# dusk-network/dusk-blindbidproof

Hardware: AMD Instinct MI355X
Metric: blind-bid proofs/sec (higher is better)
Workload: dtype u32

## Files before the change

__graft_entry__.py:

```python
import os
import shutil
import subprocess
import sys

ROOT = os.path.dirname(os.path.abspath(__file__))
PKG = os.path.join(ROOT, "dusk_blindbidproof_amd")
CSRC = os.path.join(PKG, "csrc")
LIB = os.path.join(PKG, "libbbp_hip.so")
ORACLE_SO = os.path.join(ROOT, "oracle", "_build", "libbbp_oracle.so")
HOSTCHECK_SO = os.path.join(ROOT, "tests", "_build", "libhostcheck.so")
DEVCHECK_SO = {"chain": os.path.join(ROOT, "tests", "_build", "libbbp_devcheck.so"),
               "nochain": os.path.join(ROOT, "tests", "_build", "libbbp_devcheck_nochain.so")}
DEVCHECK_DEFS = {"chain": [], "nochain": ["-DBBP_FE_NO_CHAIN"]}


def _newer(target, sources):
    if not os.path.exists(target):
        return True
    t = os.path.getmtime(target)
    return any(os.path.getmtime(s) > t for s in sources)


def _run(cmd):
    print("+", " ".join(cmd), flush=True)
# ... 273 lines not shown
        _run(["g++", "-O1", "-g", "-std=c++17", "-fsanitize=address,undefined", "-fno-sanitize-recover=all", "-o", ROUND_STANDING_BIN, src])
    return ROUND_STANDING_BIN


ROUNDS_BEST_DISTINCT_BIN = os.path.join(ROOT, "tests", "_build", "rounds_best_distinct_check")


def build_rounds_best_distinct_check(force=False):
    src = os.path.join(ROOT, "tests", "rounds_best_distinct_check.cpp")
    if force or _newer(ROUNDS_BEST_DISTINCT_BIN, [src] + _csrc_files((".h", ".inc")) + [os.path.join(ROOT, "include", "bbp.h")]):
        os.makedirs(os.path.dirname(ROUNDS_BEST_DISTINCT_BIN), exist_ok=True)
        _run(["g++", "-O1", "-g", "-std=c++17", "-fsanitize=address,undefined", "-fno-sanitize-recover=all", "-o", ROUNDS_BEST_DISTINCT_BIN, src])
    return ROUNDS_BEST_DISTINCT_BIN


def build_secret_wipe_san(force=False):
    srcs = [os.path.join(ROOT, "tests", "secret_wipe_san.cpp"), os.path.join(CSRC, "submit.cpp")]
    if force or _newer(SECRET_WIPE_SAN_BIN, srcs + _csrc_files((".h", ".inc"))):
        os.makedirs(os.path.dirname(SECRET_WIPE_SAN_BIN), exist_ok=True)
        _run(["g++", "-O1", "-g", "-std=c++17", "-pthread", "-fsanitize=address,undefined", "-fno-sanitize-recover=all", "-o", SECRET_WIPE_SAN_BIN] + srcs)
    return SECRET_WIPE_SAN_BIN


STUB_ENTROPY_SO = os.path.join(ROOT, "tests", "_build", "libbbp_stub_entropy.so")


def build_stub_engine_entropy(force=False):
    srcs = [os.path.join(ROOT, "tests", "stub_engine_entropy.cpp"), os.path.join(CSRC, "submit.cpp")]
    if force or _newer(STUB_ENTROPY_SO, srcs + [os.path.join(ROOT, "tests", "stub_engine.cpp"), os.path.join(CSRC, "submit.h"), os.path.join(ROOT, "include", "bbp.h")]):
        os.makedirs(os.path.dirname(STUB_ENTROPY_SO), exist_ok=True)
# ... 51 lines not shown

def build():
    build_hip()
    build_server()
    build_stub_engine()
    build_oracle()
    build_hostcheck()
    build_sortcheck()
    build_roundcheck()
    build_round_select_check()
    build_round_best_check()
    build_round_best_distinct_check()
    build_rounds_best_check()
    build_rounds_best_distinct_check()
    build_round_standing_check()
    build_devcheck_all()
    sys.path.insert(0, ROOT)
    import dusk_blindbidproof_amd


def smoke():
    sys.path.insert(0, ROOT)
    import dusk_blindbidproof_amd as bbp
    from tests import smoke_case

    smoke_case.run(bbp)


if __name__ == "__main__":
    build()
# ... 1 lines not shown
```

dusk_blindbidproof_amd/csrc/msm.hip:

```cpp
#include "context.h"

namespace bbp {

#ifndef BBP_FOLD_PRIO
#define BBP_FOLD_PRIO 2
#endif
#ifndef BBP_MSM_WAVES
#define BBP_MSM_WAVES 2
#endif
#ifndef BBP_MSM_WAVES_MAX
#define BBP_MSM_WAVES_MAX 2
#endif

#ifdef BBP_MSM_PROF
__device__ unsigned long long g_msm_prof[8];
#define MSM_PROF_BEGIN() unsigned long long prof_t = wall_clock64()
#define MSM_PROF_MARK(i)                                                    \
    if (tid == 0) {                                                         \
        unsigned long long now_ = wall_clock64();                           \
        atomicAdd(&g_msm_prof[i], now_ - prof_t);                           \
        prof_t = now_;                                                      \
    }
#else
#define MSM_PROF_BEGIN()
// ... 60 lines not shown
    const u32 An = A ^ (neg << 6);
    const uint4 a0 = *reinterpret_cast<const uint4*>(wb + An), a1 = *reinterpret_cast<const uint4*>(wb + (An ^ 0x10u));
    const uint2 a2 = *reinterpret_cast<const uint2*>(wb + (An ^ 0x20u));
    const uint4 b0 = *reinterpret_cast<const uint4*>(wb + (An ^ 0x40u)), b1 = *reinterpret_cast<const uint4*>(wb + (An ^ 0x50u));
    const uint2 b2 = *reinterpret_cast<const uint2*>(wb + (An ^ 0x60u));
    const uint2 x0 = *reinterpret_cast<const uint2*>(wb + (A ^ 0x20u) + 8);
    const uint4 x1 = *reinterpret_cast<const uint4*>(wb + (A ^ 0x30u));
    const uint2 x2 = *reinterpret_cast<const uint2*>(wb + (A ^ 0x60u) + 8), x3 = *reinterpret_cast<const uint2*>(wb + (A ^ 0x70u));
    row_regs r;
    r.ypx = fe{{(i32)a0.x, (i32)a0.y, (i32)a0.z, (i32)a0.w, (i32)a1.x, (i32)a1.y, (i32)a1.z, (i32)a1.w, (i32)a2.x, (i32)a2.y}};
    r.ymx = fe{{(i32)b0.x, (i32)b0.y, (i32)b0.z, (i32)b0.w, (i32)b1.x, (i32)b1.y, (i32)b1.z, (i32)b1.w, (i32)b2.x, (i32)b2.y}};
    r.xy2d = fe{{(i32)x0.x, (i32)x0.y, (i32)x1.x, (i32)x1.y, (i32)x1.z, (i32)x1.w, (i32)x2.x, (i32)x2.y, (i32)x3.x, (i32)x3.y}};
    return r;
}
#endif

__device__ __noinline__ void ge_add_nc(ge& r, const ge& a, const ge& b) { r = ge_add(a, b); }
__device__ __noinline__ void ge_dbl_nc(ge& r, const ge& a) { r = ge_dbl(a); }

#ifndef BBP_SORT_T
#define BBP_SORT_T 1024
#endif
constexpr int SORT_T = BBP_SORT_T;
template <int MODE> struct msm_geom;
template <> struct msm_geom<0> { static constexpr int K = MSM_K, NAF = MSM_NAF, W = MSM_W; };
template <> struct msm_geom<1> { static constexpr int K = FOLD_K, NAF = FOLD_NAF, W = FOLD_W; };
template <> struct msm_geom<2> { static constexpr int K = SMALL_K, NAF = SMALL_NAF, W = SMALL_W; };

template <int MODE>
__global__ __launch_bounds__(SORT_T) void k_msm_sort(const u32* __restrict__ scal_a, const u32* __restrict__ aux, u32 n_total, u32 n_idx_sets,
                                                      u32 n_sub, u32 split, u32* __restrict__ sorted_all, u32* __restrict__ cursor_all,
                                                      const u32* __restrict__ msm_map, const u32* __restrict__ n_active, u32* __restrict__ ticket) {
    constexpr int K = msm_geom<MODE>::K, NAF = msm_geom<MODE>::NAF, W = msm_geom<MODE>::W, G = K >= SORT_T ? K / SORT_T : 1;
// ... 259 lines not shown
        __syncthreads();
    }
    u32* cur_out = cursor_all + work * (size_t)(K + 1);
    for (int k = tid; k <= K; k += SORT_T) cur_out[k] = k ? start[k + 1] : 0u;
}

#ifndef BBP_ACC_WG
#define BBP_ACC_WG 256
#endif
constexpr int ACC_WG = BBP_ACC_WG, ACC_WGS = ACC_T / ACC_WG;
static_assert(ACC_T % ACC_WG == 0 && ACC_WG % 64 == 0, "accumulate workgroup geometry");

template <int MODE>
__global__ __launch_bounds__(ACC_WG) __attribute__((amdgpu_waves_per_eu(BBP_MSM_WAVES, BBP_MSM_WAVES_MAX)))
void k_msm_acc(const niels_row* __restrict__ ptable, const u32* __restrict__ sorted_all, const u32* __restrict__ cursor_all, u32 n ,
               ge* __restrict__ bsum_all, ge* __restrict__ psum_all, ge* __restrict__ out, const u32* __restrict__ n_active, u32* __restrict__ fault,
               u32 n_work, u32* __restrict__ ticket) {
    constexpr int K = msm_geom<MODE>::K, W = msm_geom<MODE>::W, G = K / MSM_T;
    __shared__ u32 cursor[K + 1];
#ifdef BBP_ACC_PERSIST
    static_assert(ACC_WGS == 1, "the persistent form draws whole MSMs");
    __shared__ u32 s_ticket;
  for (;;) {
    __syncthreads();
    if (threadIdx.x == 0) s_ticket = atomicAdd(ticket, 1u);
    __syncthreads();
    const size_t msm = s_ticket;
    if (msm >= n_work || (n_active && msm >= *n_active)) return;
    const int tid = (int)threadIdx.x;
#else
    const size_t msm = blockIdx.x / ACC_WGS;
    const int tid = (int)(blockIdx.x % ACC_WGS) * ACC_WG + (int)threadIdx.x;
// ... 2 lines not shown
    const u32* sorted = sorted_all + msm * (size_t)n * W;
#ifdef BBP_MSM_PRIO
    __builtin_amdgcn_s_setprio(BBP_MSM_PRIO);
#endif
    MSM_PROF_BEGIN();
    {
        const u32* cur_in = cursor_all + msm * (size_t)(K + 1);
        for (int k = threadIdx.x; k <= K; k += ACC_WG) cursor[k] = cur_in[k];
    }
    __syncthreads();
    MSM_PROF_MARK(1);

    const u32 E = cursor[K];
    ge* bsum = bsum_all + msm * (size_t)K;
    ge* psum = psum_all + msm * (size_t)ACC_T;
#ifdef BBP_KO_ACC_PERMILLE
    const u32 c0 = (u32)(((u64)tid * E) / ACC_T), c1 = c0 + (u32)(((u64)((u32)(((u64)(tid + 1) * E) / ACC_T) - c0) * BBP_KO_ACC_PERMILLE) / 1000);
#else
    const u32 c0 = (u32)(((u64)tid * E) / ACC_T), c1 = (u32)(((u64)(tid + 1) * E) / ACC_T);
#endif
#ifdef BBP_MSM_PROF
    const unsigned long long clk0 = clock64();
#endif
    u32 k_first = 0;
    bool inside = false;
#ifdef BBP_ACC_COOP
    {
        __shared__ __attribute__((aligned(1024))) u8 rowimg[ACC_WG / 64][COOP_IMG];
        const int lane = (int)threadIdx.x & 63;
        u8* wb = rowimg[threadIdx.x >> 6];
// ... 1 lines not shown
        const u32 srcoff = (((u32)lane & 7u) ^ (((u32)lane >> 3) >> 1)) << 4;
        const u32 n_it = (E + (u32)ACC_T - 1) / (u32)ACC_T, len = c1 - c0;
        u32 k = 1, kend = 0;
        ge* dest = &psum[tid];
        if (len) {
            u32 lo = 1, hi = K;
            while (lo < hi) {
                u32 mid = (lo + hi) >> 1;
                if (cursor[mid] > c0) hi = mid; else lo = mid + 1;
            }
            k = lo, kend = cursor[k];
            k_first = lo;
            inside = cursor[k - 1] < c0;
            if (!inside) dest = &bsum[k - 1];
        }
        ge acc = ge_identity();
        u32 ent_cur = len ? sorted[c0] : 0u;
        u32 ent_nxt = len > 1 ? sorted[c0 + 1] : 0u;
        if (n_it) coop_issue(ptable, wb, coop_clamp_row(ent_cur, fault), lane, srcoff);
        for (u32 it = 0; it < n_it; it++) {
            const u32 e = c0 + it;
            const row_regs cur = coop_read(wb, A, ent_cur >> 31);
            const bool neg = ent_cur >> 31;
            ent_cur = ent_nxt;
            const bool live = it < len;
            if (live && e == kend) {
                *dest = acc;
                acc = ge_identity();
                do { k++; kend = cursor[k]; } while (kend == e);
                dest = &bsum[k - 1];
// ... 3 lines not shown
            if (it + 2 < len) ent_nxt = sorted[e + 2]; else ent_nxt = 0u;
            if (live) acc = ge_madd_row(acc, cur, neg);
        }
        if (len) *dest = acc;
    }
#else
    if (c0 < c1) {
        u32 lo = 1, hi = K;
        while (lo < hi) {
            u32 mid = (lo + hi) >> 1;
            if (cursor[mid] > c0) hi = mid; else lo = mid + 1;
        }
        u32 k = lo, kend = cursor[k];
        k_first = lo;
        inside = cursor[k - 1] < c0;
        ge* dest = inside ? &psum[tid] : &bsum[k - 1];
        ge acc = ge_identity();
        u32 ent_cur = sorted[c0];
        u32 ent_nxt = (c0 + 1 < c1) ? sorted[c0 + 1] : 0u;
        row_regs row = load_row(ptable, ent_cur, fault);
        for (u32 e = c0; e < c1; e++) {
            if (e == kend) {
                *dest = acc;
                acc = ge_identity();
                do { k++; kend = cursor[k]; } while (kend == e);
                dest = &bsum[k - 1];
            }
            const row_regs cur = row;
            const bool neg = ent_cur >> 31;
            ent_cur = ent_nxt;
            if (e + 1 < c1) row = load_row(ptable, ent_cur, fault);
            if (e + 2 < c1) ent_nxt = sorted[e + 2];
            acc = ge_madd_row(acc, cur, neg);
        }
        *dest = acc;
    }
#endif
#ifdef BBP_MSM_PROF
    if (tid == 0) atomicAdd(&g_msm_prof[6], clock64() - clk0);
#endif
    MSM_PROF_MARK(2);
    __threadfence_block();
    __syncthreads();
    MSM_PROF_MARK(3);
#ifdef BBP_ACC_PERSIST
  }
#endif
}

template <int MODE>
__global__ __launch_bounds__(MSM_T) void k_msm_fold(const u32* __restrict__ cursor_all, ge* __restrict__ bsum_all, const ge* __restrict__ psum_all,
                                                     ge* __restrict__ out, const u32* __restrict__ n_active) {
    constexpr int K = msm_geom<MODE>::K, G = K / MSM_T;
    __shared__ u32 cursor[K + 1];
    __shared__ u32 xch[GE_WORDS];
    const int tid = threadIdx.x;
    if (n_active && blockIdx.x >= *n_active) return;
    __builtin_amdgcn_s_setprio(BBP_FOLD_PRIO);
    const size_t msm = blockIdx.x;
    {
        const u32* cur_in = cursor_all + msm * (size_t)(K + 1);
        for (int k = tid; k <= K; k += MSM_T) cursor[k] = cur_in[k];
    }
    __syncthreads();
    const u32 E = cursor[K];
    ge* bsum = bsum_all + msm * (size_t)K;
    const ge* psum = psum_all + msm * (size_t)ACC_T;
#ifdef BBP_KO_FOLD
    if (MODE != 1) { if (tid == 0) out[msm] = bsum[0]; }
    else if (tid < FOLD_CLS) out[msm * FOLD_CLS + tid] = bsum[tid];
    return;
#endif
    for (u32 ch = tid; ch < (u32)ACC_T; ch += MSM_T) {
        const u32 c0 = (u32)(((u64)ch * E) / ACC_T), c1 = (u32)(((u64)(ch + 1) * E) / ACC_T);
        if (c0 >= c1) continue;
        u32 lo = 1, hi = K;
        while (lo < hi) {
            u32 mid = (lo + hi) >> 1;
            if (cursor[mid] > c0) hi = mid; else lo = mid + 1;
        }
        const u32 k_first = lo;
        const bool inside = cursor[lo - 1] < c0;
        const bool last_of_run = inside && !(c1 < E && c1 > cursor[k_first - 1] && c1 < cursor[k_first]);
        if (last_of_run) {
            ge part = psum[ch];
            for (int u = (int)ch - 1; u >= 0; u--) {
                const u32 cu = (u32)(((u64)u * E) / ACC_T), cu1 = (u32)(((u64)(u + 1) * E) / ACC_T);
                if (cu <= cursor[k_first - 1]) break;
                if (cu1 > cu) ge_add_nc(part, part, psum[u]);
            }
            ge head = bsum[k_first - 1];
            ge_add_nc(head, head, part);
            bsum[k_first - 1] = head;
        }
    }
    __threadfence_block();
    __syncthreads();

    ge running = ge_identity(), total = ge_identity();
    if constexpr (G == 1) {
        if (cursor[tid + 1] != cursor[tid]) running = bsum[tid];
        total = running;
    } else {
#pragma unroll 1
        for (int r = G; r >= 1; r--) {
            const u32 k = tid * G + r;
            if (cursor[k] != cursor[k - 1]) running = ge_add(running, bsum[k - 1]);
            total = ge_add(total, running);
        }
    }

    if constexpr (MODE != 1) {
        const int lane = tid & 63, wave = tid >> 6;
#pragma unroll 1
        for (int d = 1; d < 64; d <<= 1) {
            ge other = ge_shfl_down(running, d);
            if (lane + d < 64) running = ge_add(running, other);
        }
        if (MSM_T > 64) {
            if (tid == 64) xch_put(xch, running);
            __syncthreads();
            if (wave == 0) {
                ge other = xch_get(xch);
                ge_add_nc(running, running, other);
            }
        }
        ge x = total;
        if (tid >= 1) {
            ge s = running;
            constexpr int LOG_G = G == 1 ? 0 : G == 2 ? 1 : G == 4 ? 2 : G == 8 ? 3 : G == 16 ? 4 : -1;
            static_assert(LOG_G >= 0, "buckets per fold lane must be a power of two up to 16");
            for (int i = 0; i < LOG_G; i++) ge_dbl_nc(s, s);
            ge_add_nc(x, x, s);
        }
#pragma unroll 1
        for (int d = 32; d >= 1; d >>= 1) {
            ge other = ge_shfl_down(x, d);
            if (lane < d) x = ge_add(x, other);
        }
        if (MSM_T > 64) {
            __syncthreads();
            if (tid == 64) xch_put(xch, x);
            __syncthreads();
        }
        if (tid == 0) {
            if (MSM_T > 64) {
                ge other = xch_get(xch);
                ge_add_nc(x, x, other);
            }
            ge other;
            ge_dbl_nc(x, x);
            other = ge_neg(running);
            ge_add_nc(x, x, other);
            out[msm] = x;
        }
    } else {
        constexpr int LPC = FOLD_M / G, LOG_G2 = G == 32 ? 5 : 6;
        static_assert(G == 32 || G == 64, "class reduction written for 4 or 2 lanes per class");
        const int q = tid & (LPC - 1);
        ge suf = running;
        for (int d = 1; d < LPC; d++) {
            ge other = ge_shfl_down(running, d);
            if (q + d < LPC) ge_add_nc(suf, suf, other);
        }
        ge x = total;
        if (q >= 1) {
            ge sg = suf;
            for (int i = 0; i < LOG_G2; i++) ge_dbl_nc(sg, sg);
            ge_add_nc(x, x, sg);
        }
        ge accq = x;
        for (int d = 1; d < LPC; d++) {
            ge other = ge_shfl_down(x, d);
            if (q == 0) ge_add_nc(accq, accq, other);
        }
        if (q == 0) {
            ge_dbl_nc(accq, accq);
            ge other = ge_neg(suf);
            ge_add_nc(accq, accq, other);
            out[msm * FOLD_CLS + (tid / LPC)] = accq;
        }
    }
}

constexpr int FOLD2_L = 32;
constexpr int FOLD2_G = MSM_K / FOLD2_L;
constexpr int FOLD2_LOG_G = 5;
static_assert(FOLD2_G == 32 && ACC_T % FOLD2_L == 0, "fold geometry");

__device__ __forceinline__ ge ge_shfl_down32(const ge& p, int d) {
    ge r;
    const u32* w = reinterpret_cast<const u32*>(&p);
    u32* o = reinterpret_cast<u32*>(&r);
#pragma unroll
    for (int i = 0; i < GE_WORDS; i++) o[i] = (u32)__shfl_down((int)w[i], d, 32);
    return r;
}

__device__ __forceinline__ ge ge_add_t2d(const ge& p, const fe& p2d, const ge& q) {
    fe a = fe_mul(fe_sub(p.Y, p.X), fe_sub(q.Y, q.X));
    fe b = fe_mul(fe_add(p.Y, p.X), fe_add(q.Y, q.X));
    fe c = fe_mul(p2d, q.T);
    fe zz = fe_mul(p.Z, q.Z);
    fe d = fe_add(zz, zz);
    fe e = fe_sub(b, a), f = fe_sub(d, c), g = fe_add(d, c), h = fe_add(b, a);
    ge r;
    r.X = fe_mul(e, f);
    r.Y = fe_mul(g, h);
    r.Z = fe_mul(g, f);
    r.T = fe_mul(e, h);
    return r;
}

__device__ __forceinline__ void park_put(u32* park, int tid, const ge& p) {
    const u32* w = reinterpret_cast<const u32*>(&p);
#pragma unroll
    for (int i = 0; i < GE_WORDS; i++) park[i * 64 + tid] = w[i];
}

__device__ __forceinline__ ge park_get(const u32* park, int tid) {
    ge p;
    u32* w = reinterpret_cast<u32*>(&p);
#pragma unroll
    for (int i = 0; i < GE_WORDS; i++) w[i] = park[i * 64 + tid];
    return p;
}

__device__ __forceinline__ ge ld_ge(const ge* p) {
    ge r;
    const uint4* s = reinterpret_cast<const uint4*>(p);
    u32* o = reinterpret_cast<u32*>(&r);
#pragma unroll
    for (int i = 0; i < GE_WORDS / 4; i++) {
        const uint4 v = s[i];
        o[4 * i] = v.x, o[4 * i + 1] = v.y, o[4 * i + 2] = v.z, o[4 * i + 3] = v.w;
    }
    return r;
}

#ifndef BBP_FOLD_WAVES
#define BBP_FOLD_WAVES 2
#endif
__global__ __launch_bounds__(64) __attribute__((amdgpu_waves_per_eu(BBP_FOLD_WAVES, BBP_FOLD_WAVES))) void k_msm_fold_half(const u32* __restrict__ cursor_all, ge* __restrict__ bsum_all, const ge* __restrict__ psum_all,
                                                       ge* __restrict__ out, u32 n_work, const u32* __restrict__ n_active) {
    constexpr int K = MSM_K, G = FOLD2_G;
    __shared__ u32 cursor2[2][K + 1];
    __shared__ u32 park[GE_WORDS * 64];
    const int tid = threadIdx.x, half = tid >> 5, l = tid & 31;
    const u32 n_tot = n_active ? min(*n_active, n_work) : n_work;
    if (2u * blockIdx.x >= n_tot) return;
    __builtin_amdgcn_s_setprio(BBP_FOLD_PRIO);
    const size_t msm = 2 * (size_t)blockIdx.x + half;
    const bool valid = msm < n_tot;
    u32* cursor = cursor2[half];
    {
        const u32* cur_in = cursor_all + msm * (size_t)(K + 1);
        for (int k = l; k <= K; k += FOLD2_L) cursor[k] = valid ? cur_in[k] : 0u;
    }
    __syncthreads();
    const u32 E = cursor[K];
    ge* bsum = bsum_all + (valid ? msm : 0) * (size_t)K;
    const ge* psum = psum_all + (valid ? msm : 0) * (size_t)ACC_T;
#pragma unroll 1
    for (u32 ch = l; ch < (u32)ACC_T; ch += FOLD2_L) {
        const u32 c0 = (u32)(((u64)ch * E) / ACC_T), c1 = (u32)(((u64)(ch + 1) * E) / ACC_T);
        bool last_of_run = false;
        u32 k_first = 1;
        if (c0 < c1) {
            u32 lo = 1, hi = K;
            while (lo < hi) {
                u32 mid = (lo + hi) >> 1;
                if (cursor[mid] > c0) hi = mid; else lo = mid + 1;
            }
            k_first = lo;
            const bool inside = cursor[lo - 1] < c0;
            last_of_run = inside && !(c1 < E && c1 > cursor[k_first - 1] && c1 < cursor[k_first]);
        }
        if (last_of_run) {
            ge part = ld_ge(&psum[ch]);
            for (int u = (int)ch - 1; u >= 0; u--) {
                const u32 cu = (u32)(((u64)u * E) / ACC_T), cu1 = (u32)(((u64)(u + 1) * E) / ACC_T);
                if (cu <= cursor[k_first - 1]) break;
                if (cu1 > cu) {
                    const ge more = ld_ge(&psum[u]);
                    part = ge_add(part, more);
                }
            }
            const ge head = ld_ge(&bsum[k_first - 1]);
            bsum[k_first - 1] = ge_add(head, part);
        }
    }
    __threadfence_block();
    __syncthreads();

    ge running = ge_identity();
    fe r2d = fe_zero();
    park_put(park, tid, ge_identity());
#pragma unroll 1
    for (int r = G; r >= 1; r--) {
        const u32 k = (u32)l * G + r;
        if (cursor[k] != cursor[k - 1]) {
            const ge cur = ld_ge(&bsum[k - 1]);
            running = ge_add_t2d(running, r2d, cur);
            r2d = fe_mul(running.T, fe_d2());
        }
        const ge total = park_get(park, tid);
        park_put(park, tid, ge_add_t2d(running, r2d, total));
    }

    ge v = running;
#pragma unroll 1
    for (int it = 0; it < 12; it++) {
        ge q;
        bool take;
        int n_dbl = 0;
        if (it == 5) {
            q = v;
            v = park_get(park, tid);
            park_put(park, tid, q);
            n_dbl = FOLD2_LOG_G;
            take = l >= 1;
        } else if (it == 11) {
            q = ge_neg(park_get(park, tid));
            take = true;
        } else {
            const int d = it < 5 ? (1 << it) : (16 >> (it - 6));
            q = ge_shfl_down32(v, d);
            take = it < 5 ? (l + d < 32) : (l < d);
        }
        if (it == 11) {
            v = ge_dbl(v);
        } else {
#pragma unroll 1
            for (int i = 0; i < n_dbl; i++) q = ge_dbl(q);
        }
        if (take) v = ge_add(v, q);
    }
    if (l == 0 && valid) out[msm] = v;
}

constexpr int REDUCE_L = 16;
__global__ __launch_bounds__(64) void k_msm_reduce(u32 n_out, u32 split, u32 items, const ge* __restrict__ tmp, ge* __restrict__ out) {
    __builtin_amdgcn_s_setprio(3);
    const u32 t = blockIdx.x * blockDim.x + threadIdx.x;
    const u32 o = t / REDUCE_L, j = t % REDUCE_L;
    const u32 msm = o / items, c = o % items;
    ge acc = ge_identity();
    if (o < n_out && j < split) acc = tmp[((size_t)msm * split + j) * items + c];
    for (u32 jj = j + REDUCE_L; o < n_out && jj < split; jj += REDUCE_L)
        acc = ge_add(acc, tmp[((size_t)msm * split + jj) * items + c]);
#pragma unroll 1
    for (int d = REDUCE_L / 2; d >= 1; d >>= 1) {
        const ge other = ge_shfl_down(acc, d);
        if ((int)j < d) acc = ge_add(acc, other);
    }
    if (o < n_out && j == 0) out[o] = acc;
}


struct MsmScratch {
    u32 *sorted, *cursor;
    ge *bsum, *psum, *tmp;
    u32* ticket;
    size_t bytes;
};
static MsmScratch msm_scratch_layout(void* base, size_t n_msm, size_t n_terms, size_t W, size_t K, size_t out_items = 1) {
    auto up = [](size_t x) { return (x + 255) / 256 * 256; };
    MsmScratch m;
    size_t o = 0;
    m.sorted = reinterpret_cast<u32*>(static_cast<u8*>(base) + o);
    o += up(n_msm * n_terms * W * sizeof(u32));
    m.cursor = reinterpret_cast<u32*>(static_cast<u8*>(base) + o);
    o += up(n_msm * (K + 1) * sizeof(u32));
    m.bsum = reinterpret_cast<ge*>(static_cast<u8*>(base) + o);
    o += n_msm * K * sizeof(ge);
    m.psum = reinterpret_cast<ge*>(static_cast<u8*>(base) + o);
    o += n_msm * ACC_T * sizeof(ge);
    m.tmp = reinterpret_cast<ge*>(static_cast<u8*>(base) + o);
    o += up(n_msm * out_items * sizeof(ge));
    m.ticket = reinterpret_cast<u32*>(static_cast<u8*>(base) + o);
    o += 256;
    m.bytes = o;
    return m;
}
size_t msm_scratch_bytes(uint32_t n_msm, uint32_t n_terms) {
    const u32 split = msm_split(n_msm, n_terms), n_sub = (n_terms + split - 1) / split;
    size_t a = msm_scratch_layout(nullptr, (size_t)n_msm * split, n_sub, MSM_W, MSM_K).bytes;
    if (split > 1) a = std::max(a, msm_scratch_layout(nullptr, (size_t)n_msm * split, n_sub, SMALL_W, SMALL_K).bytes);
    const size_t b = msm_scratch_layout(nullptr, n_msm, n_terms, MSM_W, MSM_K).bytes;
    return a > b ? a : b;
}

// ... 21 lines not shown
        if (ctx->msm_knobs.sort_staged & 2) {
            if (!ctx->sort_lds_attr1) {
                BBP_HIP_TRY(ctx, hipFuncSetAttribute((const void*)k_msm_sort_staged<1, SORT_S_FOLD>, hipFuncAttributeMaxDynamicSharedMemorySize, (int)(sort_cap<1>::V * 4)));
                ctx->sort_lds_attr1 = true;
            }
            hipLaunchKernelGGL((k_msm_sort_staged<1, SORT_S_FOLD>), dim3((u32)n_work), dim3(SORT_T), sort_cap<1>::V * 4, stream, (const u32*)g_dev, (const u32*)h_dev, 2048u, 1u,
                               n_sub, split, m.sorted, m.cursor, (const u32*)nullptr, (const u32*)nullptr, sort_cap<1>::V, m.ticket);
        } else
            hipLaunchKernelGGL(k_msm_sort<1>, dim3((u32)n_work), dim3(SORT_T), 0, stream, (const u32*)g_dev, (const u32*)h_dev, 2048u, 1u, n_sub, split,
                               m.sorted, m.cursor, (const u32*)nullptr, (const u32*)nullptr, m.ticket);
        BBP_HIP_TRY(ctx, hipGetLastError());
    }
    {
        ScopedEvent ev(ctx, TAG_MSM, stream);
        hipLaunchKernelGGL(k_msm_acc<1>, dim3(acc_grid(ctx, (u32)n_work)), dim3(ACC_WG), 0, stream, ctx->ptable, m.sorted, m.cursor, n_sub, m.bsum, m.psum,
                           split > 1 ? m.tmp : out_dev, (const u32*)nullptr, ctx->health, (u32)n_work, m.ticket);
        BBP_HIP_TRY(ctx, hipGetLastError());
    }
    ScopedEvent evf(ctx, TAG_MSM_FOLD, stream);
    hipLaunchKernelGGL(k_msm_fold<1>, dim3((u32)n_work), dim3(MSM_T), 0, stream, m.cursor, m.bsum, m.psum, split > 1 ? m.tmp : out_dev,
                       (const u32*)nullptr);
    BBP_HIP_TRY(ctx, hipGetLastError());
    if (split > 1) {
        const u32 n_out = (u32)n_msm * FOLD_CLS;
        hipLaunchKernelGGL(k_msm_reduce, dim3((n_out * REDUCE_L + 63) / 64), dim3(64), lds_token(ctx), stream, n_out, split, (u32)FOLD_CLS, m.tmp, out_dev);
        BBP_HIP_TRY(ctx, hipGetLastError());
    }
    return BBP_OK;
}

__global__ __launch_bounds__(64) void k_encode(const ge* __restrict__ pts, u32 n, u32* __restrict__ out_words) {
    u32 i = blockIdx.x * blockDim.x + threadIdx.x;
    if (i >= n) return;
    ge p = pts[i];
    u32 w[8];
// ... 21 lines not shown
    if (plan.geom == MsmPlan::SMALL) {
        const MsmScratch ms = msm_scratch_layout(scratch.p, n_work, n_sub, SMALL_W, SMALL_K);
        {
            ScopedEvent ev(ctx, TAG_MSM_SORT, stream);
            hipLaunchKernelGGL(k_msm_sort<2>, dim3(n_work), dim3(SORT_T), 0, stream, scalars_dev, base_idx_dev, n_terms, n_idx_sets, n_sub, split, ms.sorted, ms.cursor,
                               msm_map_dev, n_active_dev, ms.ticket);
            BBP_HIP_TRY(ctx, hipGetLastError());
        }
        if (ctx->debug_corrupt) {
            ctx->debug_corrupt = 0;
            hipLaunchKernelGGL(k_debug_poke, dim3(1), dim3(1), 0, stream, ms.sorted);
            BBP_HIP_TRY(ctx, hipGetLastError());
        }
        {
            ScopedEvent ev(ctx, TAG_MSM, stream);
            hipLaunchKernelGGL(k_msm_acc<2>, dim3(acc_grid(ctx, n_work)), dim3(ACC_WG), 0, stream, ctx->ptable, ms.sorted, ms.cursor, n_sub, ms.bsum, ms.psum, ms.tmp,
                               n_active_dev, ctx->health, n_work, ms.ticket);
            BBP_HIP_TRY(ctx, hipGetLastError());
        }
        {
            ScopedEvent evf(ctx, TAG_MSM_FOLD, stream);
            hipLaunchKernelGGL(k_msm_fold<2>, dim3(n_work), dim3(MSM_T), 0, stream, ms.cursor, ms.bsum, ms.psum, ms.tmp, n_active_dev);
            BBP_HIP_TRY(ctx, hipGetLastError());
        }
        hipLaunchKernelGGL(k_msm_reduce, dim3((n_msm * REDUCE_L + 63) / 64), dim3(64), lds_token(ctx), stream, n_msm, split, 1u, ms.tmp, out_points_dev);
        BBP_HIP_TRY(ctx, hipGetLastError());
        return BBP_OK;
    }
    const MsmScratch m = msm_scratch_layout(scratch.p, n_work, n_sub, MSM_W, MSM_K);
    {
        ScopedEvent ev(ctx, TAG_MSM_SORT, stream);
        if (plan.sort != MsmPlan::PLAIN) {
            const u32 cap = plan.sort_cap;
            if (!ctx->sort_lds_attr) {
                BBP_HIP_TRY(ctx, hipFuncSetAttribute((const void*)k_msm_sort_staged<0, SORT_S>, hipFuncAttributeMaxDynamicSharedMemorySize, (int)(SORT_CAP_WIDE * 4)));
                BBP_HIP_TRY(ctx, hipFuncSetAttribute((const void*)k_msm_sort_staged<0, SORT_S_WIDE>, hipFuncAttributeMaxDynamicSharedMemorySize, (int)(SORT_CAP_WIDE * 4)));
                ctx->sort_lds_attr = true;
// ... 13 lines not shown
            hipLaunchKernelGGL(k_msm_sort<0>, dim3(n_work), dim3(SORT_T), 0, stream, scalars_dev, base_idx_dev, n_terms, n_idx_sets, n_sub, split,
                               m.sorted, m.cursor, msm_map_dev, n_active_dev, m.ticket);
        BBP_HIP_TRY(ctx, hipGetLastError());
    }
    if (ctx->debug_corrupt) {
        ctx->debug_corrupt = 0;
        hipLaunchKernelGGL(k_debug_poke, dim3(1), dim3(1), 0, stream, m.sorted);
        BBP_HIP_TRY(ctx, hipGetLastError());
    }
    chain_acc = chain_acc && ctx->verify_serial_acc;
    if (chain_acc && ctx->vacc_valid)
        BBP_HIP_TRY(ctx, hipStreamWaitEvent(stream, ctx->ev_vacc[ctx->vacc_seq % bbp_ctx::VACC_RING], 0));
    {
        ScopedEvent ev(ctx, TAG_MSM, stream);
        hipLaunchKernelGGL(k_msm_acc<0>, dim3(acc_grid(ctx, n_work)), dim3(ACC_WG), 0, stream, ctx->ptable, m.sorted, m.cursor, n_sub, m.bsum, m.psum,
                           split > 1 ? m.tmp : out_points_dev, n_active_dev, ctx->health, n_work, m.ticket);
        BBP_HIP_TRY(ctx, hipGetLastError());
    }
    static const bool chain_after_fold = getenv("BBP_VERIFY_CHAIN_AFTER_FOLD") && atoi(getenv("BBP_VERIFY_CHAIN_AFTER_FOLD"));
    if (chain_acc && !chain_after_fold) {
        ctx->vacc_seq++;
        BBP_HIP_TRY(ctx, hipEventRecord(ctx->ev_vacc[ctx->vacc_seq % bbp_ctx::VACC_RING], stream));
        ctx->vacc_valid = true;
    }
    ScopedEvent evf(ctx, TAG_MSM_FOLD, stream);
    if (plan.fold == MsmPlan::HALF)
        hipLaunchKernelGGL(k_msm_fold_half, dim3((n_work + 1) / 2), dim3(64), 0, stream, m.cursor, m.bsum, m.psum, split > 1 ? m.tmp : out_points_dev,
                           n_work, n_active_dev);
    else
        hipLaunchKernelGGL(k_msm_fold<0>, dim3(n_work), dim3(MSM_T), 0, stream, m.cursor, m.bsum, m.psum, split > 1 ? m.tmp : out_points_dev, n_active_dev);
    BBP_HIP_TRY(ctx, hipGetLastError());
    if (chain_acc && chain_after_fold) {
        ctx->vacc_seq++;
        BBP_HIP_TRY(ctx, hipEventRecord(ctx->ev_vacc[ctx->vacc_seq % bbp_ctx::VACC_RING], stream));
        ctx->vacc_valid = true;
    }
    if (plan.reduce) {
        hipLaunchKernelGGL(k_msm_reduce, dim3((n_msm * REDUCE_L + 63) / 64), dim3(64), lds_token(ctx), stream, n_msm, split, 1u, m.tmp, out_points_dev);
        BBP_HIP_TRY(ctx, hipGetLastError());
    }
#ifdef BBP_MSM_PROF
    static int launches = 0;
    if (++launches % 16 == 0) {
        unsigned long long h[8], sp[4][16];
        (void)hipStreamSynchronize(stream);
// ... 25 lines not shown
```

dusk_blindbidproof_amd/csrc/msm_plan.h:

```cpp
#pragma once
#include <stdint.h>
#include <stdlib.h>
#include <string.h>

#include <initializer_list>

namespace bbp {

constexpr int MSM_NAF = 12;
constexpr int MSM_W = 22;
constexpr int MSM_K = 1 << (MSM_NAF - 2);
constexpr int SMALL_NAF = 9;
constexpr int SMALL_K = 1 << (SMALL_NAF - 2);
constexpr int SMALL_W = 29;

#ifndef BBP_SORT_CAP
#define BBP_SORT_CAP 21504
#endif
constexpr uint32_t SORT_CAP_WIDE = 32768;
constexpr uint32_t SORT_WIDE_FROM = 3000;
constexpr uint32_t SORT_STAGED_MAX_TERMS = 5120;
constexpr uint32_t MSM_SPLIT_MAX = 16;

struct MsmKnobs {
// ... 27 lines not shown
        for (const char* name : {"BBP_SORT_STAGED", "BBP_FOLD_HALF_FROM", "BBP_MSM_SMALL"})
            if (const char* text = getenv(name)) k.set(name, text);
        return k;
    }
};

inline uint32_t msm_split(const MsmKnobs& k, uint32_t n_msm, uint32_t n_terms) {
    if (n_msm >= k.split_below) return 1;
    uint32_t s = k.split_target / n_msm;
    if (s > MSM_SPLIT_MAX) s = MSM_SPLIT_MAX;
    while (s > 1 && n_terms / s < 128) s--;
    return s ? s : 1;
}
inline uint32_t msm_split(uint32_t n_msm, uint32_t n_terms) { return msm_split(MsmKnobs::process(), n_msm, n_terms); }

struct MsmPlan {
    enum Geom { LARGE, SMALL };
    enum Sort { PLAIN, STAGED, STAGED_WIDE };
    enum Fold { LANES128, HALF, SMALL_FOLD };
    uint32_t split = 1;
    uint32_t n_sub = 0;
    uint32_t n_work = 0;
    Geom geom = LARGE;
    Sort sort = PLAIN;
    uint32_t sort_cap = 0;
    Fold fold = LANES128;
    bool reduce = false;

    uint32_t K() const { return geom == SMALL ? SMALL_K : MSM_K; }
    uint32_t W() const { return geom == SMALL ? SMALL_W : MSM_W; }
// ... 25 lines not shown
```

Baseline: 23230.

## Tag chunks in accumulate kernel and prefetch fold buckets into LDS

The accumulate kernel now writes a per-chunk tag (first bucket plus inside flag), so the fold kernels no longer redo the binary search over cursors to find run boundaries. The half fold replaces its cursor LDS copy with a ballot-built occupancy mask, prefetches the next bucket point into LDS with global_load_lds while computing the current one, and reduces across lanes through LDS instead of shuffles. Noinline add/dbl wrappers are inlined and a VGPR cap is added. This costs an extra tag buffer, some global writes, and a linear tag scan in place of the binary search, and it risks register spills under the new VGPR cap.

```diff
diff --git a/__graft_entry__.py b/__graft_entry__.py
--- a/__graft_entry__.py
+++ b/__graft_entry__.py
@@ -311,6 +311,17 @@
     return ROUNDS_BEST_DISTINCT_BIN
 
 
+MSM_TAGS_BIN = os.path.join(ROOT, "tests", "_build", "msm_tags_check")
+
+
+def build_msm_tags_check(force=False):
+    src = os.path.join(ROOT, "tests", "msm_tags_check.cpp")
+    if force or _newer(MSM_TAGS_BIN, [src, os.path.join(CSRC, "msm_plan.h")]):
+        os.makedirs(os.path.dirname(MSM_TAGS_BIN), exist_ok=True)
+        _run(["g++", "-O1", "-g", "-std=c++17", "-fsanitize=address,undefined", "-fno-sanitize-recover=all", "-o", MSM_TAGS_BIN, src])
+    return MSM_TAGS_BIN
+
+
 def build_secret_wipe_san(force=False):
     srcs = [os.path.join(ROOT, "tests", "secret_wipe_san.cpp"), os.path.join(CSRC, "submit.cpp")]
     if force or _newer(SECRET_WIPE_SAN_BIN, srcs + _csrc_files((".h", ".inc"))):
@@ -392,6 +403,7 @@
     build_rounds_best_check()
     build_rounds_best_distinct_check()
     build_round_standing_check()
+    build_msm_tags_check()
     build_devcheck_all()
     sys.path.insert(0, ROOT)
     import dusk_blindbidproof_amd
diff --git a/dusk_blindbidproof_amd/csrc/msm.hip b/dusk_blindbidproof_amd/csrc/msm.hip
--- a/dusk_blindbidproof_amd/csrc/msm.hip
+++ b/dusk_blindbidproof_amd/csrc/msm.hip
@@ -98,9 +98,6 @@
     return r;
 }
 #endif
-
-__device__ __noinline__ void ge_add_nc(ge& r, const ge& a, const ge& b) { r = ge_add(a, b); }
-__device__ __noinline__ void ge_dbl_nc(ge& r, const ge& a) { r = ge_dbl(a); }
 
 #ifndef BBP_SORT_T
 #define BBP_SORT_T 1024
@@ -390,8 +387,8 @@
 template <int MODE>
 __global__ __launch_bounds__(ACC_WG) __attribute__((amdgpu_waves_per_eu(BBP_MSM_WAVES, BBP_MSM_WAVES_MAX)))
 void k_msm_acc(const niels_row* __restrict__ ptable, const u32* __restrict__ sorted_all, const u32* __restrict__ cursor_all, u32 n ,
-               ge* __restrict__ bsum_all, ge* __restrict__ psum_all, ge* __restrict__ out, const u32* __restrict__ n_active, u32* __restrict__ fault,
-               u32 n_work, u32* __restrict__ ticket) {
+               ge* __restrict__ bsum_all, ge* __restrict__ psum_all, u32* __restrict__ tag_all, ge* __restrict__ out, const u32* __restrict__ n_active,
+               u32* __restrict__ fault, u32 n_work, u32* __restrict__ ticket) {
     constexpr int K = msm_geom<MODE>::K, W = msm_geom<MODE>::W, G = K / MSM_T;
     __shared__ u32 cursor[K + 1];
 #ifdef BBP_ACC_PERSIST
@@ -424,6 +421,7 @@
     const u32 E = cursor[K];
     ge* bsum = bsum_all + msm * (size_t)K;
     ge* psum = psum_all + msm * (size_t)ACC_T;
+    u32* tags = tag_all + msm * (size_t)ACC_T;
 #ifdef BBP_KO_ACC_PERMILLE
     const u32 c0 = (u32)(((u64)tid * E) / ACC_T), c1 = c0 + (u32)(((u64)((u32)(((u64)(tid + 1) * E) / ACC_T) - c0) * BBP_KO_ACC_PERMILLE) / 1000);
 #else
@@ -455,6 +453,7 @@
             inside = cursor[k - 1] < c0;
             if (!inside) dest = &bsum[k - 1];
         }
+        tags[tid] = len ? msm_chunk_tag(k_first, inside) : MSM_TAG_EMPTY;
         ge acc = ge_identity();
         u32 ent_cur = len ? sorted[c0] : 0u;
         u32 ent_nxt = len > 1 ? sorted[c0 + 1] : 0u;
@@ -488,6 +487,7 @@
         u32 k = lo, kend = cursor[k];
         k_first = lo;
         inside = cursor[k - 1] < c0;
+        tags[tid] = msm_chunk_tag(k_first, inside);
         ge* dest = inside ? &psum[tid] : &bsum[k - 1];
         ge acc = ge_identity();
         u32 ent_cur = sorted[c0];
@@ -508,7 +508,8 @@
             acc = ge_madd_row(acc, cur, neg);
         }
         *dest = acc;
-    }
+    } else
+        tags[tid] = MSM_TAG_EMPTY;
 #endif
 #ifdef BBP_MSM_PROF
     if (tid == 0) atomicAdd(&g_msm_prof[6], clock64() - clk0);
@@ -524,9 +525,10 @@
 
 template <int MODE>
 __global__ __launch_bounds__(MSM_T) void k_msm_fold(const u32* __restrict__ cursor_all, ge* __restrict__ bsum_all, const ge* __restrict__ psum_all,
-                                                     ge* __restrict__ out, const u32* __restrict__ n_active) {
+                                                     const u32* __restrict__ tag_all, ge* __restrict__ out, const u32* __restrict__ n_active) {
     constexpr int K = msm_geom<MODE>::K, G = K / MSM_T;
     __shared__ u32 cursor[K + 1];
+    __shared__ u32 tags[ACC_T];
     __shared__ u32 xch[GE_WORDS];
     const int tid = threadIdx.x;
     if (n_active && blockIdx.x >= *n_active) return;
@@ -535,9 +537,10 @@
     {
         const u32* cur_in = cursor_all + msm * (size_t)(K + 1);
         for (int k = tid; k <= K; k += MSM_T) cursor[k] = cur_in[k];
-    }
-    __syncthreads();
-    const u32 E = cursor[K];
+        const u32* tag_in = tag_all + msm * (size_t)ACC_T;
+        for (int ch = tid; ch < ACC_T; ch += MSM_T) tags[ch] = tag_in[ch];
+    }
+    __syncthreads();
     ge* bsum = bsum_all + msm * (size_t)K;
     const ge* psum = psum_all + msm * (size_t)ACC_T;
 #ifdef BBP_KO_FOLD
@@ -546,27 +549,12 @@
     return;
 #endif
     for (u32 ch = tid; ch < (u32)ACC_T; ch += MSM_T) {
-        const u32 c0 = (u32)(((u64)ch * E) / ACC_T), c1 = (u32)(((u64)(ch + 1) * E) / ACC_T);
-        if (c0 >= c1) continue;
-        u32 lo = 1, hi = K;
-        while (lo < hi) {
-            u32 mid = (lo + hi) >> 1;
-            if (cursor[mid] > c0) hi = mid; else lo = mid + 1;
-        }
-        const u32 k_first = lo;
-        const bool inside = cursor[lo - 1] < c0;
-        const bool last_of_run = inside && !(c1 < E && c1 > cursor[k_first - 1] && c1 < cursor[k_first]);
-        if (last_of_run) {
-            ge part = psum[ch];
-            for (int u = (int)ch - 1; u >= 0; u--) {
-                const u32 cu = (u32)(((u64)u * E) / ACC_T), cu1 = (u32)(((u64)(u + 1) * E) / ACC_T);
-                if (cu <= cursor[k_first - 1]) break;
-                if (cu1 > cu) ge_add_nc(part, part, psum[u]);
-            }
-            ge head = bsum[k_first - 1];
-            ge_add_nc(head, head, part);
-            bsum[k_first - 1] = head;
-        }
+        const u32 t = tags[ch];
+        if (!msm_tag_last_of_run(tags, (u32)ACC_T, ch, t)) continue;
+        const u32 k_first = min(max(msm_tag_bucket(t), 1u), (u32)K);
+        ge part = psum[ch];
+        for (int u = msm_tag_run_prev(tags, (int)ch, t); u >= 0; u = msm_tag_run_prev(tags, u, t)) part = ge_add(part, psum[u]);
+        bsum[k_first - 1] = ge_add(bsum[k_first - 1], part);
     }
     __threadfence_block();
     __syncthreads();
@@ -596,7 +584,7 @@
             __syncthreads();
             if (wave == 0) {
                 ge other = xch_get(xch);
-                ge_add_nc(running, running, other);
+                running = ge_add(running, other);
             }
         }
         ge x = total;
@@ -604,8 +592,8 @@
             ge s = running;
             constexpr int LOG_G = G == 1 ? 0 : G == 2 ? 1 : G == 4 ? 2 : G == 8 ? 3 : G == 16 ? 4 : -1;
             static_assert(LOG_G >= 0, "buckets per fold lane must be a power of two up to 16");
-            for (int i = 0; i < LOG_G; i++) ge_dbl_nc(s, s);
-            ge_add_nc(x, x, s);
+            for (int i = 0; i < LOG_G; i++) s = ge_dbl(s);
+            x = ge_add(x, s);
         }
 #pragma unroll 1
         for (int d = 32; d >= 1; d >>= 1) {
@@ -620,12 +608,12 @@
         if (tid == 0) {
             if (MSM_T > 64) {
                 ge other = xch_get(xch);
-                ge_add_nc(x, x, other);
+                x = ge_add(x, other);
             }
             ge other;
-            ge_dbl_nc(x, x);
+            x = ge_dbl(x);
             other = ge_neg(running);
-            ge_add_nc(x, x, other);
+            x = ge_add(x, other);
             out[msm] = x;
         }
     } else {
@@ -635,23 +623,23 @@
         ge suf = running;
         for (int d = 1; d < LPC; d++) {
             ge other = ge_shfl_down(running, d);
-            if (q + d < LPC) ge_add_nc(suf, suf, other);
+            if (q + d < LPC) suf = ge_add(suf, other);
         }
         ge x = total;
         if (q >= 1) {
             ge sg = suf;
-            for (int i = 0; i < LOG_G2; i++) ge_dbl_nc(sg, sg);
-            ge_add_nc(x, x, sg);
+            for (int i = 0; i < LOG_G2; i++) sg = ge_dbl(sg);
+            x = ge_add(x, sg);
         }
         ge accq = x;
         for (int d = 1; d < LPC; d++) {
             ge other = ge_shfl_down(x, d);
-            if (q == 0) ge_add_nc(accq, accq, other);
+            if (q == 0) accq = ge_add(accq, other);
         }
         if (q == 0) {
-            ge_dbl_nc(accq, accq);
+            accq = ge_dbl(accq);
             ge other = ge_neg(suf);
-            ge_add_nc(accq, accq, other);
+            accq = ge_add(accq, other);
             out[msm * FOLD_CLS + (tid / LPC)] = accq;
         }
     }
@@ -662,27 +650,36 @@
 constexpr int FOLD2_LOG_G = 5;
 static_assert(FOLD2_G == 32 && ACC_T % FOLD2_L == 0, "fold geometry");
 
-__device__ __forceinline__ ge ge_shfl_down32(const ge& p, int d) {
-    ge r;
-    const u32* w = reinterpret_cast<const u32*>(&p);
-    u32* o = reinterpret_cast<u32*>(&r);
-#pragma unroll
-    for (int i = 0; i < GE_WORDS; i++) o[i] = (u32)__shfl_down((int)w[i], d, 32);
-    return r;
-}
-
-__device__ __forceinline__ ge ge_add_t2d(const ge& p, const fe& p2d, const ge& q) {
-    fe a = fe_mul(fe_sub(p.Y, p.X), fe_sub(q.Y, q.X));
-    fe b = fe_mul(fe_add(p.Y, p.X), fe_add(q.Y, q.X));
-    fe c = fe_mul(p2d, q.T);
-    fe zz = fe_mul(p.Z, q.Z);
+template <class Rd, class Put>
+__device__ __forceinline__ void ge_add_t2d_lds_put(const ge& p, const fe& p2d, Rd rd, Put put) {
+    auto coord = [&](int c) {
+        fe v;
+#pragma unroll
+        for (int i = 0; i < 10; i++) v.v[i] = (i32)rd(10 * c + i);
+        return v;
+    };
+    fe a, b;
+    {
+        const fe qx = coord(0), qy = coord(1);
+        a = fe_mul(fe_sub(p.Y, p.X), fe_sub(qy, qx));
+        b = fe_mul(fe_add(p.Y, p.X), fe_add(qy, qx));
+    }
+    asm volatile("" ::: "memory");
+    fe c = fe_mul(p2d, coord(3));
+    asm volatile("" ::: "memory");
+    fe zz = fe_mul(p.Z, coord(2));
+    asm volatile("" ::: "memory");
     fe d = fe_add(zz, zz);
     fe e = fe_sub(b, a), f = fe_sub(d, c), g = fe_add(d, c), h = fe_add(b, a);
+    put(0, fe_mul(e, f));
+    put(1, fe_mul(g, h));
+    put(2, fe_mul(g, f));
+    put(3, fe_mul(e, h));
+}
+template <class Rd>
+__device__ __forceinline__ ge ge_add_t2d_lds(const ge& p, const fe& p2d, Rd rd) {
     ge r;
-    r.X = fe_mul(e, f);
-    r.Y = fe_mul(g, h);
-    r.Z = fe_mul(g, f);
-    r.T = fe_mul(e, h);
+    ge_add_t2d_lds_put(p, p2d, rd, [&](int c, const fe& v) { (c == 0 ? r.X : c == 1 ? r.Y : c == 2 ? r.Z : r.T) = v; });
     return r;
 }
 
@@ -712,53 +709,53 @@
     return r;
 }
 
+__device__ __forceinline__ void pref_issue(u32* pref, const ge* src) {
+    const u8* g = reinterpret_cast<const u8*>(src);
+#pragma unroll
+    for (int i = 0; i < GE_WORDS / 4; i++)
+        __builtin_amdgcn_global_load_lds((const __attribute__((address_space(1))) void*)(g + 16 * i), (__attribute__((address_space(3))) void*)(pref + i * 256), 16, 0, 0);
+}
+
 #ifndef BBP_FOLD_WAVES
 #define BBP_FOLD_WAVES 2
 #endif
-__global__ __launch_bounds__(64) __attribute__((amdgpu_waves_per_eu(BBP_FOLD_WAVES, BBP_FOLD_WAVES))) void k_msm_fold_half(const u32* __restrict__ cursor_all, ge* __restrict__ bsum_all, const ge* __restrict__ psum_all,
-                                                       ge* __restrict__ out, u32 n_work, const u32* __restrict__ n_active) {
+#ifndef BBP_FOLD_VGPRS
+#define BBP_FOLD_VGPRS 192
+#endif
+__global__ __launch_bounds__(64) __attribute__((amdgpu_waves_per_eu(BBP_FOLD_WAVES, BBP_FOLD_WAVES), amdgpu_num_vgpr(BBP_FOLD_VGPRS / 2)))
+void k_msm_fold_half(const u32* __restrict__ cursor_all, ge* __restrict__ bsum_all, const ge* __restrict__ psum_all, const u32* __restrict__ tag_all,
+                     ge* __restrict__ out, u32 n_work, const u32* __restrict__ n_active) {
     constexpr int K = MSM_K, G = FOLD2_G;
-    __shared__ u32 cursor2[2][K + 1];
     __shared__ u32 park[GE_WORDS * 64];
+    __shared__ __attribute__((aligned(16))) u32 pref[GE_WORDS * 64];
     const int tid = threadIdx.x, half = tid >> 5, l = tid & 31;
     const u32 n_tot = n_active ? min(*n_active, n_work) : n_work;
     if (2u * blockIdx.x >= n_tot) return;
     __builtin_amdgcn_s_setprio(BBP_FOLD_PRIO);
     const size_t msm = 2 * (size_t)blockIdx.x + half;
     const bool valid = msm < n_tot;
-    u32* cursor = cursor2[half];
-    {
-        const u32* cur_in = cursor_all + msm * (size_t)(K + 1);
-        for (int k = l; k <= K; k += FOLD2_L) cursor[k] = valid ? cur_in[k] : 0u;
-    }
-    __syncthreads();
-    const u32 E = cursor[K];
     ge* bsum = bsum_all + (valid ? msm : 0) * (size_t)K;
     const ge* psum = psum_all + (valid ? msm : 0) * (size_t)ACC_T;
+    const u32* tags = tag_all + (valid ? msm : 0) * (size_t)ACC_T;
+    u32 full = 0;
+    {
+        const u32* cur_in = cursor_all + (valid ? msm : 0) * (size_t)(K + 1);
+#pragma unroll 4
+        for (int j = 0; j < K / FOLD2_L; j++) {
+            const u32 k = (u32)(j * FOLD2_L + l + 1);
+            const unsigned long long b = __ballot(valid && cur_in[k] != cur_in[k - 1]);
+            if (l == j) full = half ? (u32)(b >> 32) : (u32)b;
+        }
+    }
 #pragma unroll 1
     for (u32 ch = l; ch < (u32)ACC_T; ch += FOLD2_L) {
-        const u32 c0 = (u32)(((u64)ch * E) / ACC_T), c1 = (u32)(((u64)(ch + 1) * E) / ACC_T);
-        bool last_of_run = false;
-        u32 k_first = 1;
-        if (c0 < c1) {
-            u32 lo = 1, hi = K;
-            while (lo < hi) {
-                u32 mid = (lo + hi) >> 1;
-                if (cursor[mid] > c0) hi = mid; else lo = mid + 1;
-            }
-            k_first = lo;
-            const bool inside = cursor[lo - 1] < c0;
-            last_of_run = inside && !(c1 < E && c1 > cursor[k_first - 1] && c1 < cursor[k_first]);
-        }
-        if (last_of_run) {
+        const u32 t = valid ? tags[ch] : MSM_TAG_EMPTY;
+        if (msm_tag_last_of_run(tags, (u32)ACC_T, ch, t)) {
+            const u32 k_first = min(max(msm_tag_bucket(t), 1u), (u32)K);
             ge part = ld_ge(&psum[ch]);
-            for (int u = (int)ch - 1; u >= 0; u--) {
-                const u32 cu = (u32)(((u64)u * E) / ACC_T), cu1 = (u32)(((u64)(u + 1) * E) / ACC_T);
-                if (cu <= cursor[k_first - 1]) break;
-                if (cu1 > cu) {
-                    const ge more = ld_ge(&psum[u]);
-                    part = ge_add(part, more);
-                }
+            for (int u = msm_tag_run_prev(tags, (int)ch, t); u >= 0; u = msm_tag_run_prev(tags, u, t)) {
+                const ge more = ld_ge(&psum[u]);
+                part = ge_add(part, more);
             }
             const ge head = ld_ge(&bsum[k_first - 1]);
             bsum[k_first - 1] = ge_add(head, part);
@@ -770,47 +767,51 @@
     ge running = ge_identity();
     fe r2d = fe_zero();
     park_put(park, tid, ge_identity());
+    if (full >> (G - 1) & 1) pref_issue(pref, &bsum[(u32)l * G + G - 1]);
 #pragma unroll 1
     for (int r = G; r >= 1; r--) {
-        const u32 k = (u32)l * G + r;
-        if (cursor[k] != cursor[k - 1]) {
-            const ge cur = ld_ge(&bsum[k - 1]);
-            running = ge_add_t2d(running, r2d, cur);
+        if (full >> (r - 1) & 1) {
+            asm volatile("s_waitcnt vmcnt(0)" ::: "memory");
+            running = ge_add_t2d_lds(running, r2d, [&](int w) { return pref[(w >> 2) * 256 + 4 * tid + (w & 3)]; });
             r2d = fe_mul(running.T, fe_d2());
-        }
-        const ge total = park_get(park, tid);
-        park_put(park, tid, ge_add_t2d(running, r2d, total));
+            asm volatile("s_waitcnt lgkmcnt(0)" ::: "memory");
+        }
+        if (r > 1 && (full >> (r - 2) & 1)) pref_issue(pref, &bsum[(u32)l * G + r - 2]);
+        ge_add_t2d_lds_put(running, r2d, [&](int w) { return park[w * 64 + tid]; }, [&](int c, const fe& v) {
+#pragma unroll
+            for (int i = 0; i < 10; i++) park[(10 * c + i) * 64 + tid] = (u32)v.v[i];
+            asm volatile("" ::: "memory");
+        });
     }
 
     ge v = running;
 #pragma unroll 1
     for (int it = 0; it < 12; it++) {
-        ge q;
-        bool take;
-        int n_dbl = 0;
+        const u32* slot = it < 5 || it == 11 ? pref : park;
+        int from = tid, n_dbl = 0;
+        bool take = true;
         if (it == 5) {
-            q = v;
-            v = park_get(park, tid);
-            park_put(park, tid, q);
+            park_put(pref, tid, ge_neg(v));
             n_dbl = FOLD2_LOG_G;
             take = l >= 1;
+            slot = park;
         } else if (it == 11) {
-            q = ge_neg(park_get(park, tid));
-            take = true;
+            n_dbl = 1;
         } else {
             const int d = it < 5 ? (1 << it) : (16 >> (it - 6));
-            q = ge_shfl_down32(v, d);
+            park_put(it < 5 ? pref : park, tid, v);
+            from = tid + d;
             take = it < 5 ? (l + d < 32) : (l < d);
         }
-        if (it == 11) {
-            v = ge_dbl(v);
-        } else {
 #pragma unroll 1
-            for (int i = 0; i < n_dbl; i++) q = ge_dbl(q);
-        }
-        if (take) v = ge_add(v, q);
-    }
-    if (l == 0 && valid) out[msm] = v;
+        for (int i = 0; i < n_dbl; i++) v = ge_dbl(v);
+        if (take) v = ge_add_t2d_lds(v, fe_mul(v.T, fe_d2()), [&](int w) { return slot[w * 64 + from]; });
+        else if (it == 5) v = park_get(park, tid);
+    }
+    if ((threadIdx.x & 31) == 0) {
+        const size_t mine = 2 * (size_t)blockIdx.x + (threadIdx.x >> 5);
+        if (mine < n_tot) out[mine] = v;
+    }
 }
 
 constexpr int REDUCE_L = 16;
@@ -835,6 +836,7 @@
 struct MsmScratch {
     u32 *sorted, *cursor;
     ge *bsum, *psum, *tmp;
+    u32* tags;
     u32* ticket;
     size_t bytes;
 };
@@ -850,6 +852,8 @@
     o += n_msm * K * sizeof(ge);
     m.psum = reinterpret_cast<ge*>(static_cast<u8*>(base) + o);
     o += n_msm * ACC_T * sizeof(ge);
+    m.tags = reinterpret_cast<u32*>(static_cast<u8*>(base) + o);
+    o += up(n_msm * ACC_T * sizeof(u32));
     m.tmp = reinterpret_cast<ge*>(static_cast<u8*>(base) + o);
     o += up(n_msm * out_items * sizeof(ge));
     m.ticket = reinterpret_cast<u32*>(static_cast<u8*>(base) + o);
@@ -901,11 +905,11 @@
     {
         ScopedEvent ev(ctx, TAG_MSM, stream);
         hipLaunchKernelGGL(k_msm_acc<1>, dim3(acc_grid(ctx, (u32)n_work)), dim3(ACC_WG), 0, stream, ctx->ptable, m.sorted, m.cursor, n_sub, m.bsum, m.psum,
-                           split > 1 ? m.tmp : out_dev, (const u32*)nullptr, ctx->health, (u32)n_work, m.ticket);
+                           m.tags, split > 1 ? m.tmp : out_dev, (const u32*)nullptr, ctx->health, (u32)n_work, m.ticket);
         BBP_HIP_TRY(ctx, hipGetLastError());
     }
     ScopedEvent evf(ctx, TAG_MSM_FOLD, stream);
-    hipLaunchKernelGGL(k_msm_fold<1>, dim3((u32)n_work), dim3(MSM_T), 0, stream, m.cursor, m.bsum, m.psum, split > 1 ? m.tmp : out_dev,
+    hipLaunchKernelGGL(k_msm_fold<1>, dim3((u32)n_work), dim3(MSM_T), 0, stream, m.cursor, m.bsum, m.psum, m.tags, split > 1 ? m.tmp : out_dev,
                        (const u32*)nullptr);
     BBP_HIP_TRY(ctx, hipGetLastError());
     if (split > 1) {
@@ -957,13 +961,13 @@
         }
         {
             ScopedEvent ev(ctx, TAG_MSM, stream);
-            hipLaunchKernelGGL(k_msm_acc<2>, dim3(acc_grid(ctx, n_work)), dim3(ACC_WG), 0, stream, ctx->ptable, ms.sorted, ms.cursor, n_sub, ms.bsum, ms.psum, ms.tmp,
+            hipLaunchKernelGGL(k_msm_acc<2>, dim3(acc_grid(ctx, n_work)), dim3(ACC_WG), 0, stream, ctx->ptable, ms.sorted, ms.cursor, n_sub, ms.bsum, ms.psum, ms.tags, ms.tmp,
                                n_active_dev, ctx->health, n_work, ms.ticket);
             BBP_HIP_TRY(ctx, hipGetLastError());
         }
         {
             ScopedEvent evf(ctx, TAG_MSM_FOLD, stream);
-            hipLaunchKernelGGL(k_msm_fold<2>, dim3(n_work), dim3(MSM_T), 0, stream, ms.cursor, ms.bsum, ms.psum, ms.tmp, n_active_dev);
+            hipLaunchKernelGGL(k_msm_fold<2>, dim3(n_work), dim3(MSM_T), 0, stream, ms.cursor, ms.bsum, ms.psum, ms.tags, ms.tmp, n_active_dev);
             BBP_HIP_TRY(ctx, hipGetLastError());
         }
         hipLaunchKernelGGL(k_msm_reduce, dim3((n_msm * REDUCE_L + 63) / 64), dim3(64), lds_token(ctx), stream, n_msm, split, 1u, ms.tmp, out_points_dev);
@@ -1007,7 +1011,7 @@
     {
         ScopedEvent ev(ctx, TAG_MSM, stream);
         hipLaunchKernelGGL(k_msm_acc<0>, dim3(acc_grid(ctx, n_work)), dim3(ACC_WG), 0, stream, ctx->ptable, m.sorted, m.cursor, n_sub, m.bsum, m.psum,
-                           split > 1 ? m.tmp : out_points_dev, n_active_dev, ctx->health, n_work, m.ticket);
+                           m.tags, split > 1 ? m.tmp : out_points_dev, n_active_dev, ctx->health, n_work, m.ticket);
         BBP_HIP_TRY(ctx, hipGetLastError());
     }
     static const bool chain_after_fold = getenv("BBP_VERIFY_CHAIN_AFTER_FOLD") && atoi(getenv("BBP_VERIFY_CHAIN_AFTER_FOLD"));
@@ -1018,10 +1022,10 @@
     }
     ScopedEvent evf(ctx, TAG_MSM_FOLD, stream);
     if (plan.fold == MsmPlan::HALF)
-        hipLaunchKernelGGL(k_msm_fold_half, dim3((n_work + 1) / 2), dim3(64), 0, stream, m.cursor, m.bsum, m.psum, split > 1 ? m.tmp : out_points_dev,
+        hipLaunchKernelGGL(k_msm_fold_half, dim3((n_work + 1) / 2), dim3(64), 0, stream, m.cursor, m.bsum, m.psum, m.tags, split > 1 ? m.tmp : out_points_dev,
                            n_work, n_active_dev);
     else
-        hipLaunchKernelGGL(k_msm_fold<0>, dim3(n_work), dim3(MSM_T), 0, stream, m.cursor, m.bsum, m.psum, split > 1 ? m.tmp : out_points_dev, n_active_dev);
+        hipLaunchKernelGGL(k_msm_fold<0>, dim3(n_work), dim3(MSM_T), 0, stream, m.cursor, m.bsum, m.psum, m.tags, split > 1 ? m.tmp : out_points_dev, n_active_dev);
     BBP_HIP_TRY(ctx, hipGetLastError());
     if (chain_acc && chain_after_fold) {
         ctx->vacc_seq++;
diff --git a/dusk_blindbidproof_amd/csrc/msm_plan.h b/dusk_blindbidproof_amd/csrc/msm_plan.h
--- a/dusk_blindbidproof_amd/csrc/msm_plan.h
+++ b/dusk_blindbidproof_amd/csrc/msm_plan.h
@@ -65,6 +65,36 @@
 }
 inline uint32_t msm_split(uint32_t n_msm, uint32_t n_terms) { return msm_split(MsmKnobs::process(), n_msm, n_terms); }
 
+constexpr uint32_t MSM_TAG_EMPTY = 0;
+constexpr uint32_t MSM_TAG_INSIDE = 1u << 31;
+constexpr uint32_t msm_chunk_begin(uint32_t ch, uint32_t E, uint32_t T) { return (uint32_t)(((uint64_t)ch * E) / T); }
+constexpr uint32_t msm_bucket_of(const uint32_t* cursor, uint32_t K, uint32_t c) {
+    uint32_t lo = 1, hi = K;
+    while (lo < hi) {
+        const uint32_t mid = (lo + hi) >> 1;
+        if (cursor[mid] > c) hi = mid; else lo = mid + 1;
+    }
+    return lo;
+}
+constexpr uint32_t msm_chunk_tag(uint32_t k_first, bool inside) { return k_first | (inside ? MSM_TAG_INSIDE : 0u); }
+constexpr uint32_t msm_tag_bucket(uint32_t tag) { return tag & ~MSM_TAG_INSIDE; }
+constexpr bool msm_tag_inside(uint32_t tag) { return (tag & MSM_TAG_INSIDE) != 0; }
+constexpr bool msm_tag_last_of_run(const uint32_t* tags, uint32_t T, uint32_t ch, uint32_t t) {
+    if (!msm_tag_inside(t)) return false;
+    for (uint32_t v = ch + 1; v < T; v++) {
+        const uint32_t tv = tags[v];
+        if (tv != MSM_TAG_EMPTY) return tv != t;
+    }
+    return true;
+}
+constexpr int msm_tag_run_prev(const uint32_t* tags, int u, uint32_t t) {
+    for (u = u - 1; u >= 0; u--) {
+        const uint32_t tv = tags[u];
+        if (tv != MSM_TAG_EMPTY) return tv == t ? u : -1;
+    }
+    return -1;
+}
+
 struct MsmPlan {
     enum Geom { LARGE, SMALL };
     enum Sort { PLAIN, STAGED, STAGED_WIDE };
```

Result: no change. 23030 (-0.8%).
